# fugue-project/fugue

Measured on NVIDIA H100. Metric: transform() rows/sec, hash-partitioned (num=256) identity map, 8-col table, higher is better.
Workload: dtype int64+f64 (byte moves; u64 hash arithmetic)

## Files before the change

fugue_b200/csrc/fb_partition.cu:

```cuda
#include <stdlib.h>

#include <mutex>

#include "fb_common.cuh"

namespace {

constexpr int kBlock = 512;
constexpr int kItems = 8;
constexpr int kTile = kBlock * kItems;
constexpr int kWarps = kBlock / 32;
constexpr int kCtasPerSm = 2;

struct FbCols {
  const void* src[FB_MAX_COLS];
  void* dst[FB_MAX_COLS];
  int32_t width[FB_MAX_COLS];
  int32_t ncols;
};

struct ChunkGeom {
  int64_t nrows;
  int64_t full_rows;
  int64_t tiles_per_chunk;
  int32_t nchunks_full;
  int32_t nchunks;
};

inline ChunkGeom make_geom(int dev, int64_t nrows) {
  ChunkGeom g;
  g.nrows = nrows;
  const int64_t ntiles_full = nrows / kTile;
  g.full_rows = ntiles_full * kTile;
  const int64_t max_chunks = (int64_t)fb_sm_count(dev) * kCtasPerSm;
  g.tiles_per_chunk = ntiles_full > 0 ? (ntiles_full + max_chunks - 1) / max_chunks : 1;
  g.nchunks_full = (int32_t)((ntiles_full + g.tiles_per_chunk - 1) / g.tiles_per_chunk);
  g.nchunks = g.nchunks_full + (g.full_rows < nrows ? 1 : 0);
  return g;
}

__host__ __device__ __forceinline__ void chunk_range(const ChunkGeom& g, int c, int64_t& r0, int64_t& r1) {
  if (c < g.nchunks_full) {
    r0 = (int64_t)c * g.tiles_per_chunk * kTile;
    r1 = r0 + g.tiles_per_chunk * kTile;
    if (r1 > g.full_rows) r1 = g.full_rows;
  } else {
    r0 = g.full_rows;
    r1 = g.nrows;
  }
}
// ... 15 lines not shown
__global__ void fb_pid_kernel(FbKeys keys, FbDiv dv, int64_t nrows, uint32_t* __restrict__ out) {
  int64_t i = (int64_t)blockIdx.x * blockDim.x + threadIdx.x;
  int64_t stride = (int64_t)gridDim.x * blockDim.x;
  for (; i < nrows; i += stride) out[i] = compute_pid<kSingleU64>(keys, dv, i);
}

__global__ void fb_row_hash_kernel(FbKeys keys, int64_t nrows, uint64_t* __restrict__ out) {
  int64_t i = (int64_t)blockIdx.x * blockDim.x + threadIdx.x;
  int64_t stride = (int64_t)gridDim.x * blockDim.x;
  for (; i < nrows; i += stride) out[i] = fb_row_hash(keys, i);
}

template <int kBits>
__device__ __forceinline__ unsigned match_lanes(uint32_t v, unsigned m) {
#pragma unroll
  for (int b = 0; b < kBits; ++b) {
    const int s = (int)(v << (31 - b)) >> 31;
    const unsigned bal = __ballot_sync(0xFFFFFFFFu, s < 0);
    m &= ~(bal ^ (unsigned)s);
  }
  return m;
}

constexpr int kHistBlock = 1024;
constexpr int kHistWarps = kHistBlock / 32;
constexpr int kHistRows = kHistBlock * kItems;

template <bool kSingleU64, int kBits>
__global__ void __launch_bounds__(kHistBlock, 2)
fb_hist_kernel(FbKeys keys, FbDiv dv, uint32_t num, ChunkGeom g, int chunk0, uint32_t* __restrict__ hist) {
  extern __shared__ uint32_t s_cnt[];
  for (uint32_t i = threadIdx.x; i < (uint32_t)kHistWarps * num; i += kHistBlock) s_cnt[i] = 0;
  __syncthreads();
  int64_t row0, row1;
  chunk_range(g, chunk0 + (int)blockIdx.x, row0, row1);
  const unsigned lt = fb_lanemask_lt();
  uint32_t* my = s_cnt + (size_t)(threadIdx.x >> 5) * num;
  for (int64_t base = row0; base < row1; base += kHistRows) {
    uint32_t pid[kItems];
    const bool full = base + kHistRows <= row1;
#pragma unroll
    for (int r = 0; r < kItems; ++r) {
      int64_t row = base + (int64_t)r * kHistBlock + threadIdx.x;
      pid[r] = (full || row < row1) ? compute_pid<kSingleU64>(keys, dv, row) : 0xFFFFFFFFu;
    }
#pragma unroll
    for (int r = 0; r < kItems; ++r) {
      const bool ok = pid[r] != 0xFFFFFFFFu;
      unsigned m = match_lanes<kBits>(pid[r], __ballot_sync(0xFFFFFFFFu, ok));
      if (ok && (m & lt) == 0) my[pid[r]] += (uint32_t)__popc(m);
      __syncwarp();
    }
  }
  __syncthreads();
// ... 5 lines not shown
    out[b] = t;
  }
}

constexpr int kRankBlock = 512, kRankWarps = kRankBlock / 32;
constexpr int kRankRounds = kTile / 32;
constexpr int kRankBatch = 8;
constexpr uint32_t kMetaRank = kTile, kMetaCnt = 3 * kTile, kMetaBytes = 3 * kTile + 512;
static_assert(kRankRounds % kRankBatch == 0, "a tile is a whole number of key batches");

template <bool kSingleU64>
__device__ __forceinline__ uint32_t pid_of_key(const FbKeys& keys, const FbDiv& dv, uint64_t v) {
  if (kSingleU64) return fb_fastmod(fb_hash_single_u64(v), dv);
  return (uint32_t)(v >> keys.digit_shift) & (dv.d - 1);
}

template <bool kSingleU64, int kBits, bool kStaged>
__global__ void __launch_bounds__(kRankBlock, 2)
fb_rank_tile_kernel(FbKeys keys, FbDiv dv, uint32_t num, ChunkGeom g, uint32_t* __restrict__ hist,
                    uint8_t* __restrict__ meta) {
  __shared__ __align__(16) uint16_t s_cnt[kRankWarps * 256];
  __shared__ uint32_t s_hist[256];
  const unsigned lane = threadIdx.x & 31, warp = threadIdx.x >> 5;
  const unsigned lt = fb_lanemask_lt();
  uint16_t* __restrict__ my = s_cnt + warp * 256;
  ((uint4*)my)[lane] = make_uint4(0, 0, 0, 0);
  if (threadIdx.x < 256) s_hist[threadIdx.x] = 0;
  __syncthreads();
  int64_t row0, row1;
  chunk_range(g, (int)blockIdx.x, row0, row1);
  constexpr int64_t kStride = (int64_t)kRankWarps * kTile;
  uint32_t acc[8] = {0, 0, 0, 0, 0, 0, 0, 0};
  const unsigned long long* __restrict__ kp = (const unsigned long long*)keys.ptr[0] + lane;
  uint64_t kv[kRankBatch];
  if constexpr (kStaged) {
    if (row0 + (int64_t)warp * kTile < row1) {
#pragma unroll
      for (int b = 0; b < kRankBatch; ++b) kv[b] = __ldg(kp + row0 + (int64_t)warp * kTile + b * 32);
    }
  }
  for (int64_t t0 = row0 + (int64_t)warp * kTile; t0 < row1; t0 += kStride) {
    uint8_t* __restrict__ rec = meta + (size_t)(t0 / kTile) * kMetaBytes;
    uint8_t* __restrict__ rec_id = rec + lane;
    uint16_t* __restrict__ rec_rank = (uint16_t*)(rec + kMetaRank) + lane;
    for (int r0 = 0; r0 < kRankRounds; r0 += kRankBatch) {
      uint32_t pid[kRankBatch];
      if constexpr (kStaged) {
#pragma unroll
        for (int b = 0; b < kRankBatch; ++b) pid[b] = pid_of_key<kSingleU64>(keys, dv, kv[b]);
        const int64_t nxt = r0 + kRankBatch < kRankRounds ? t0 + (r0 + kRankBatch) * 32 : t0 + kStride;
        if (nxt < row1) {
#pragma unroll
          for (int b = 0; b < kRankBatch; ++b) kv[b] = __ldg(kp + nxt + b * 32);
// ... 5 lines not shown
      }
#pragma unroll
      for (int b = 0; b < kRankBatch; ++b) {
        const uint32_t p = pid[b];
        const unsigned m = match_lanes<kBits>(p, 0xFFFFFFFFu);
        const unsigned before = __popc(m & lt);
        const uint32_t old = my[p];
        __syncwarp();
        if (before == 0) my[p] = (uint16_t)(old + __popc(m));
        __syncwarp();
        rec_id[(r0 + b) * 32] = (uint8_t)p;
        rec_rank[(r0 + b) * 32] = (uint16_t)(old + before);
      }
    }
    const uint4 c = ((const uint4*)my)[lane];
    ((uint4*)(rec + kMetaCnt))[lane] = c;
    acc[0] += c.x & 0xFFFFu; acc[1] += c.x >> 16;
    acc[2] += c.y & 0xFFFFu; acc[3] += c.y >> 16;
    acc[4] += c.z & 0xFFFFu; acc[5] += c.z >> 16;
    acc[6] += c.w & 0xFFFFu; acc[7] += c.w >> 16;
    ((uint4*)my)[lane] = make_uint4(0, 0, 0, 0);
    __syncwarp();
  }
#pragma unroll
  for (int i = 0; i < 8; ++i)
    if (acc[i] != 0) atomicAdd(&s_hist[lane * 8 + i], acc[i]);
  __syncthreads();
  if (threadIdx.x < num) hist[(size_t)blockIdx.x * num + threadIdx.x] = s_hist[threadIdx.x];
}

__global__ void __launch_bounds__(256)
fb_scan_chunks_kernel(uint32_t* __restrict__ hist, uint32_t num, int32_t nchunks,
                      int64_t* __restrict__ totals) {
  __shared__ uint32_t s_warp[8];
  __shared__ uint32_t s_carry;
  const uint32_t b = blockIdx.x;
  const unsigned lane = threadIdx.x & 31, warp = threadIdx.x >> 5;
  if (threadIdx.x == 0) s_carry = 0;
  __syncthreads();
  for (int32_t c0 = 0; c0 < nchunks; c0 += 256) {
    int32_t c = c0 + threadIdx.x;
    uint32_t v = c < nchunks ? hist[(size_t)c * num + b] : 0;
    uint32_t x = v;
#pragma unroll
    for (int o = 1; o < 32; o <<= 1) {
      uint32_t y = __shfl_up_sync(0xFFFFFFFFu, x, o);
      if (lane >= (unsigned)o) x += y;
    }
    if (lane == 31) s_warp[warp] = x;
    __syncthreads();
    uint32_t wbase = 0;
    for (unsigned w = 0; w < warp; ++w) wbase += s_warp[w];
    uint32_t carry = s_carry;
    if (c < nchunks) hist[(size_t)c * num + b] = carry + wbase + x - v;
    __syncthreads();
    if (threadIdx.x == 255) s_carry = carry + wbase + x;
    __syncthreads();
  }
  if (threadIdx.x == 0) totals[b] = (int64_t)s_carry;
}

__global__ void __launch_bounds__(1024)
fb_scan_parts_kernel(int64_t* __restrict__ offsets, uint32_t num) {
  __shared__ int64_t s_warp[32];
  __shared__ int64_t s_carry;
  const unsigned lane = threadIdx.x & 31, warp = threadIdx.x >> 5;
  if (threadIdx.x == 0) s_carry = 0;
  __syncthreads();
  for (uint32_t b0 = 0; b0 < num; b0 += 1024) {
    uint32_t b = b0 + threadIdx.x;
    int64_t v = b < num ? offsets[b] : 0;
    int64_t x = v;
#pragma unroll
    for (int o = 1; o < 32; o <<= 1) {
      int64_t y = __shfl_up_sync(0xFFFFFFFFu, x, o);
      if (lane >= (unsigned)o) x += y;
    }
    if (lane == 31) s_warp[warp] = x;
    __syncthreads();
    int64_t wbase = 0;
    for (unsigned w = 0; w < warp; ++w) wbase += s_warp[w];
    int64_t carry = s_carry;
    if (b < num) offsets[b] = carry + wbase + x - v;
    __syncthreads();
    if (threadIdx.x == 1023) s_carry = carry + wbase + x;
    __syncthreads();
  }
  if (threadIdx.x == 0) offsets[num] = s_carry;
}

// ... 176 lines not shown
  cx.cursor = cx.delta + cx.nbp;
  cx.bin_start = cx.cursor + cx.nbp;
  cx.cnt = cx.bin_start + cx.nbp;
  cx.scanw = cx.cnt + kWarps * cx.nbp;
  cx.pid_sorted = (uint16_t*)(cx.scanw + 32);

  const int chunk = chunk0 + (int)blockIdx.x;
  int64_t chunk_row0, chunk_row1;
  chunk_range(g, chunk, chunk_row0, chunk_row1);

  for (uint32_t b = threadIdx.x; b < cx.nbp; b += kBlock)
    cx.cursor[b] = b < num ? (uint32_t)part_offsets[b] + chunk_base[(size_t)chunk * num + b] : 0u;
  for (uint32_t i = threadIdx.x; i < (uint32_t)kWarps * cx.nbp; i += kBlock) cx.cnt[i] = 0;
  __syncthreads();

  int phase = 0;
  for (int64_t tile_row0 = chunk_row0; tile_row0 < chunk_row1; tile_row0 += kTile) {
    const int64_t left = chunk_row1 - tile_row0;
    if (left >= kTile)
      scatter_tile<kSingleU64, kBits, true, kAll8>(keys, dv, num, cols, cx, tile_row0, kTile, phase);
    else
      scatter_tile<kSingleU64, kBits, false, kAll8>(keys, dv, num, cols, cx, tile_row0, (int)left, phase);
  }
}

constexpr int kSwcMaxCols = 8;
constexpr uint32_t kSwcMaxNum = 256;

__device__ __forceinline__ uint32_t smem_u32(const void* p) { return (uint32_t)__cvta_generic_to_shared(p); }

__device__ __forceinline__ void mbar_init(uint32_t bar, uint32_t count) {
  asm volatile("mbarrier.init.shared::cta.b64 [%0], %1;" ::"r"(bar), "r"(count) : "memory");
}
__device__ __forceinline__ void mbar_expect_tx(uint32_t bar, uint32_t bytes) {
  asm volatile("mbarrier.arrive.expect_tx.shared::cta.b64 _, [%0], %1;" ::"r"(bar), "r"(bytes) : "memory");
}
__device__ __forceinline__ void mbar_arrive_relaxed(uint32_t bar) {
  asm volatile("mbarrier.arrive.relaxed.cta.shared::cta.b64 _, [%0];" ::"r"(bar) : "memory");
}
__device__ __forceinline__ void mbar_wait(uint32_t bar, uint32_t parity) {
  asm volatile(
      "{\n"
      ".reg .pred p;\n"
      "FB_WAIT:\n"
      "mbarrier.try_wait.parity.shared::cta.b64 p, [%0], %1;\n"
      "@p bra FB_DONE;\n"
// ... 45 lines not shown
  uint64_t a[FB_MAX_COLS], b[FB_MAX_COLS], c[FB_MAX_COLS];
  int32_t mode[FB_MAX_COLS];
};

__device__ __forceinline__ uint64_t ws_apply_map(int mode, bool two, uint64_t x, uint64_t y, uint64_t a, uint64_t b,
                                                 uint64_t c) {
  if (mode == 1) {
    double r = __dmul_rn(__longlong_as_double((long long)a), __longlong_as_double((long long)x));
    if (two) r = __dadd_rn(r, __dmul_rn(__longlong_as_double((long long)b), __longlong_as_double((long long)y)));
    return (uint64_t)__double_as_longlong(__dadd_rn(r, __longlong_as_double((long long)c)));
  }
  if (mode == 2) return a * x + (two ? b * y : 0ULL) + c;
  return x;
}

template <int G, int RI>
__host__ __device__ inline size_t ws_book_bytes(uint32_t num, int ncols) {
  constexpr size_t kT = (size_t)kWsRankers * RI;
  const size_t nbp = nb_padded(num);
  const size_t E = (size_t)num * (G - 1);
  size_t b = 64 * 8;
  b += (size_t)ncols * E * 8;
  b += (kT + E) * 4;
  b += 5 * nbp * 4 + 64 * 4;
  b += ((E * 2 + 15) / 16) * 16;
  b += 2 * (size_t)kMetaBytes + 128;
  return b;
}

__device__ __forceinline__ void mbar_arrive(uint32_t bar) {
  asm volatile("mbarrier.arrive.shared::cta.b64 _, [%0];" ::"r"(bar) : "memory");
}
__device__ __forceinline__ void mover_sync() { asm volatile("bar.sync 1, %0;" ::"n"(kWsMovers) : "memory"); }
__device__ __forceinline__ void ranker_sync() { asm volatile("bar.sync 2, %0;" ::"n"(kWsRankers) : "memory"); }
template <uint32_t N>
__device__ __forceinline__ void setmaxnreg_dec() { asm volatile("setmaxnreg.dec.sync.aligned.u32 %0;" ::"n"(N)); }
template <uint32_t N>
__device__ __forceinline__ void setmaxnreg_inc() { asm volatile("setmaxnreg.inc.sync.aligned.u32 %0;" ::"n"(N)); }

template <int kBits, int G, int kWsRankItems, bool kMap>
__global__ void __launch_bounds__(kWsThreads, 1)
fb_scatter_ws_kernel(WsUnits units, uint32_t num, ChunkGeom g, int nstages,
                     const uint8_t* __restrict__ meta,
                     const uint32_t* __restrict__ chunk_base, const int64_t* __restrict__ part_offsets,
                     const __grid_constant__ WsMap map) {
  constexpr uint32_t T = (uint32_t)kWsRankers * kWsRankItems;
  static_assert(T == (uint32_t)kTile, "pass 1 ranks tiles of kTile rows");
  static_assert(G >= 2 && G <= 16 && (G & (G - 1)) == 0, "G must be a power of two <= 16");
  constexpr uint32_t GM = G - 1;
  constexpr uint32_t kStageBytes = T * 8;
  constexpr int kSlotRounds = ((int)T + (int)kSwcMaxNum * (G - 1) + kWsMovers - 1) / kWsMovers;
  constexpr int kEntryRoundsM = ((int)kSwcMaxNum * (G - 1) + kWsMovers - 1) / kWsMovers;
  extern __shared__ __align__(128) uint64_t smem64[];
  const uint32_t nbp = nb_padded(num);
  const uint32_t E = num * GM;
  const int grp = (int)blockIdx.x % units.ngroups;
  const int chunk_first = (int)blockIdx.x / units.ngroups, chunk_step = (int)gridDim.x / units.ngroups;
  const int u0 = grp * units.per_group;
  const int ncols = min(units.per_group, units.nunits - u0);
  uint64_t* ring = smem64;
  uint64_t* bars = ring + (size_t)nstages * T;
  uint64_t* carry = bars + 64;
  uint32_t* slotinfo = (uint32_t*)(carry + (size_t)ncols * E);
  uint32_t* wpos = slotinfo + T + E;
  uint32_t* kcnt = wpos + nbp;
  uint32_t* binfo = kcnt + nbp;
  uint32_t* wstart = binfo + nbp;
  uint32_t* wdelta = wstart + nbp;
  uint32_t* scanw = wdelta + nbp;
  uint16_t* carryinfo = (uint16_t*)(scanw + 64);
  uint8_t* metabuf = (uint8_t*)(((uintptr_t)(carryinfo + E) + 127) & ~(uintptr_t)127);

  const unsigned lane = threadIdx.x & 31, warp = threadIdx.x >> 5;
  const uint32_t bar_full = smem_u32(bars), bar_empty = smem_u32(bars + 16);
  const uint32_t bar_pid_full = smem_u32(bars + 32), bar_pid_empty = smem_u32(bars + 34);
  const uint32_t bar_slots_ready = smem_u32(bars + 36), bar_slots_free = smem_u32(bars + 37);
  const uint32_t bar_flush_done = smem_u32(bars + 38);

  if (threadIdx.x == 0) {
    for (int s = 0; s < nstages; ++s) {
      mbar_init(bar_full + 8 * s, 1);
      mbar_init(bar_empty + 8 * s, kWsMoverWarps);
    }
    for (int i = 0; i < 2; ++i) {
      mbar_init(bar_pid_full + 8 * i, 1);
      mbar_init(bar_pid_empty + 8 * i, kWsRankWarps);
    }
    mbar_init(bar_slots_ready, kWsRankWarps);
    mbar_init(bar_slots_free, kWsMoverWarps);
    mbar_init(bar_flush_done, kWsMoverWarps);
    asm volatile("fence.mbarrier_init.release.cluster;" ::: "memory");
  }
  __syncthreads();

  if (warp >= kWsMoverWarps + kWsRankWarps) {
    setmaxnreg_dec<kWsProducerRegs>();
    if (warp == kWsMoverWarps + kWsRankWarps && lane == 0) {
      const uint64_t pol = l2_policy_evict_first(), meta_pol = l2_policy_evict_last();
      const uint32_t ring_s = smem_u32(ring), meta_s = smem_u32(metabuf);
      uint32_t s = 0, ph = 0, seq = 0;
      int chunk = chunk_first;
      int64_t r0 = 0, r1 = 0, t0 = 0;
      bool have = chunk < g.nchunks_full;
      if (have) { chunk_range(g, chunk, r0, r1); t0 = r0; }
      auto load_pid = [&](int64_t row0, uint32_t q) {
        const uint32_t b = q & 1, pp = (q >> 1) & 1;
        mbar_wait(bar_pid_empty + 8 * b, pp ^ 1);
        mbar_expect_tx(bar_pid_full + 8 * b, kMetaBytes);
        tma_load_1d(meta_s + b * kMetaBytes, meta + (size_t)(row0 / T) * kMetaBytes, kMetaBytes,
                    bar_pid_full + 8 * b, meta_pol);
      };
      if (have) load_pid(t0, 0);
      while (have) {
        int nchunk = chunk;
        int64_t nr0 = r0, nr1 = r1, nt0 = t0 + T;
        bool nhave = true;
        if (nt0 >= r1) {
          nchunk = chunk + chunk_step;
          nhave = nchunk < g.nchunks_full;
          if (nhave) { chunk_range(g, nchunk, nr0, nr1); nt0 = nr0; }
        }
        if (nhave) load_pid(nt0, seq + 1);
        for (int u = u0; u < u0 + ncols; ++u) {
          mbar_wait(bar_empty + 8 * s, ph ^ 1);
          mbar_expect_tx(bar_full + 8 * s, kStageBytes);
          tma_load_1d(ring_s + s * kStageBytes, units.src[u] + t0, kStageBytes, bar_full + 8 * s, pol);
          if (++s == (uint32_t)nstages) { s = 0; ph ^= 1; }
          if constexpr (kMap) {
            if (map.src2[u] != nullptr) {
              mbar_wait(bar_empty + 8 * s, ph ^ 1);
              mbar_expect_tx(bar_full + 8 * s, kStageBytes);
              tma_load_1d(ring_s + s * kStageBytes, map.src2[u] + t0, kStageBytes, bar_full + 8 * s, pol);
              if (++s == (uint32_t)nstages) { s = 0; ph ^= 1; }
            }
          }
        }
        chunk = nchunk; r0 = nr0; r1 = nr1; t0 = nt0; have = nhave;
        ++seq;
      }
    }
    return;
  }

  if (warp >= kWsMoverWarps) {
    setmaxnreg_dec<kWsRankerRegs>();
    const unsigned rw = warp - kWsMoverWarps;
    const unsigned rtid = threadIdx.x - kWsMovers;
    uint32_t seq = 0, cseq = 0;
    for (int chunk = chunk_first; chunk < g.nchunks_full; chunk += chunk_step, ++cseq) {
      int64_t r0, r1;
      chunk_range(g, chunk, r0, r1);
      if (cseq > 0) mbar_wait(bar_flush_done, (cseq - 1) & 1);
      ranker_sync();
      for (uint32_t b = rtid; b < nbp; b += kWsRankers) {
        const uint32_t p0 = b < num ? (uint32_t)part_offsets[b] + chunk_base[(size_t)chunk * num + b] : 0u;
        wpos[b] = p0 & ~GM;
        kcnt[b] = (p0 & GM) | ((p0 & GM) << 8);
      }
      ranker_sync();
      for (int64_t t0 = r0; t0 < r1; t0 += T, ++seq) {
        const uint32_t pb = seq & 1, pph = (seq >> 1) & 1;
        mbar_wait(bar_pid_full + 8 * pb, pph);
        const uint8_t* __restrict__ rec = metabuf + pb * kMetaBytes;
        const uint32_t b = rtid;
        uint32_t n = 0, w = 0, kold = 0, phold = 0, wp_old = 0;
        if (b < num) n = ((const uint16_t*)(rec + kMetaCnt))[b];
        if (b < num) {
          const uint32_t kc = kcnt[b];
          kold = kc & 0xFFu;
          phold = kc >> 8;
          wp_old = wpos[b];
          const uint32_t end = wp_old + kold + n;
          const uint32_t aend = end & ~GM;
          if (aend > wp_old) {
            w = aend - wp_old;
            wpos[b] = aend;
            kcnt[b] = end - aend;
          } else {
            kcnt[b] = (kold + n) | (phold << 8);
          }
          binfo[b] = kold | (w << 8);
        }
        uint32_t xw = w;
#pragma unroll
        for (int o = 1; o < 32; o <<= 1) {
          const uint32_t yw = __shfl_up_sync(0xFFFFFFFFu, xw, o);
          if (lane >= (unsigned)o) xw += yw;
        }
        if (lane == 31) scanw[8 + rw] = xw;
        ranker_sync();
        uint32_t bw = xw - w;
        {
          const uint32_t tw = lane < kWsRankWarps ? scanw[8 + lane] : 0;
#pragma unroll
          for (int wi = 0; wi < kWsRankWarps; ++wi) {
            const uint32_t vw = __shfl_sync(0xFFFFFFFFu, tw, wi);
            if ((unsigned)wi < rw) bw += vw;
          }
        }
        if (seq > 0) mbar_wait(bar_slots_free, (seq - 1) & 1);
        if (b < num) {
          wstart[b] = bw;
          wdelta[b] = wp_old - bw;
        }
        if (rtid == kWsRankers - 1) scanw[40] = bw + w;
        ranker_sync();
#pragma unroll
        for (int r = 0; r < kWsRankItems; ++r) {
          const uint32_t row = r * kWsRankers + rtid;
          const uint32_t pb2 = rec[row];
          const uint32_t bi = binfo[pb2];
          const uint32_t i = (bi & 0xFFu) + ((const uint16_t*)(rec + kMetaRank))[row];
          const uint32_t ww = bi >> 8;
          if (i < ww) slotinfo[wstart[pb2] + i] = (pb2 << 16) | row;
          else carryinfo[pb2 * GM + (i - ww)] = (uint16_t)row;
        }
        __syncwarp();
        if (lane == 0) mbar_arrive_relaxed(bar_pid_empty + 8 * pb);
        if (b < num) {
#pragma unroll
          for (uint32_t i = 0; i < GM; ++i) {
            const uint32_t e = b * GM + i;
            const uint32_t desc = i < phold ? 0xFFFFu : T + e;
            if (i < kold) {
              if (i < w) slotinfo[bw + i] = (b << 16) | desc;
              else carryinfo[e] = (uint16_t)desc;
            }
            if (w + i >= kold + n) carryinfo[e] = 0xFFFFu;
          }
        }
        ranker_sync();
        if (lane == 0) mbar_arrive(bar_slots_ready);
      }
    }
    return;
  }

  setmaxnreg_inc<kWsMoverRegs>();
  uint32_t s = 0, ph = 0, seq = 0;
  for (int chunk = chunk_first; chunk < g.nchunks_full; chunk += chunk_step) {
    int64_t r0, r1;
    chunk_range(g, chunk, r0, r1);
    for (int64_t t0 = r0; t0 < r1; t0 += T, ++seq) {
      mbar_wait(bar_slots_ready, seq & 1);
      const uint32_t W = scanw[40];
      uint32_t srcd[kSlotRounds], dst[kSlotRounds];
#pragma unroll
      for (int k = 0; k < kSlotRounds; ++k) {
        const uint32_t j = k * kWsMovers + threadIdx.x;
        srcd[k] = 0xFFFFu;
        dst[k] = 0;
        if (j < W) {
          const uint32_t info = slotinfo[j];
          srcd[k] = info & 0xFFFFu;
          dst[k] = wdelta[info >> 16] + j;
        }
      }
      uint32_t csrc[kEntryRoundsM];
#pragma unroll
      for (int q = 0; q < kEntryRoundsM; ++q) {
        const uint32_t e = q * kWsMovers + threadIdx.x;
        const uint32_t d = e < E ? (uint32_t)carryinfo[e] : 0xFFFFu;
        csrc[q] = d < T ? d : 0xFFFFu;
      }
      __syncwarp();
      if (lane == 0) mbar_arrive(bar_slots_free);

      for (int u = 0; u < ncols; ++u) {
        mbar_wait(bar_full + 8 * s, ph);
        const uint64_t* __restrict__ st = ring + (size_t)s * T;
        uint64_t* __restrict__ out = units.dst[u0 + u];
        uint64_t* __restrict__ cbuf = carry + (size_t)u * E;
        uint32_t s2 = s;
        bool two = false;
        const uint64_t* __restrict__ st2 = st;
        int mode = 0;
        uint64_t ma = 0, mb = 0, mc = 0;
        if constexpr (kMap) {
          mode = map.mode[u0 + u];
          two = map.src2[u0 + u] != nullptr;
          if (two) {
            s2 = s + 1 == (uint32_t)nstages ? 0 : s + 1;
            mbar_wait(bar_full + 8 * s2, s2 == 0 ? ph ^ 1 : ph);
            st2 = ring + (size_t)s2 * T;
          }
          ma = map.a[u0 + u]; mb = map.b[u0 + u]; mc = map.c[u0 + u];
        }
        auto staged = [&](uint32_t r) -> uint64_t {
          if constexpr (kMap) return ws_apply_map(mode, two, st[r], st2[r], ma, mb, mc);
          else return st[r];
        };
#pragma unroll
// ... 3 lines not shown
          for (int k = 0; k < kMoveBatch; ++k)
            if (k0 + k < kSlotRounds && srcd[k0 + k] != 0xFFFFu)
              v[k] = srcd[k0 + k] < T ? staged(srcd[k0 + k]) : cbuf[srcd[k0 + k] - T];
#pragma unroll
          for (int k = 0; k < kMoveBatch; ++k)
            if (k0 + k < kSlotRounds && srcd[k0 + k] != 0xFFFFu) out[dst[k0 + k]] = v[k];
        }
        mover_sync();
#pragma unroll
        for (int q = 0; q < kEntryRoundsM; ++q)
          if (csrc[q] != 0xFFFFu) cbuf[q * kWsMovers + threadIdx.x] = staged(csrc[q]);
        __syncwarp();
        if (lane == 0) {
          mbar_arrive_relaxed(bar_empty + 8 * s);
          if (kMap && two) mbar_arrive_relaxed(bar_empty + 8 * s2);
        }
        if (++s == (uint32_t)nstages) { s = 0; ph ^= 1; }
        if (kMap && two) {
          if (++s == (uint32_t)nstages) { s = 0; ph ^= 1; }
        }
      }
      if (ncols == 1) mover_sync();
    }
    mover_sync();
    for (int u = 0; u < ncols; ++u) {
      uint64_t* __restrict__ out = units.dst[u0 + u];
      const uint64_t* __restrict__ cbuf = carry + (size_t)u * E;
#pragma unroll
      for (int q = 0; q < kEntryRoundsM; ++q) {
        const uint32_t e = q * kWsMovers + threadIdx.x;
        if (e < E) {
          const uint32_t b = e / GM, i = e - b * GM;
          const uint32_t kc = kcnt[b];
          if (i < (kc & 0xFFu) && i >= (kc >> 8)) out[wpos[b] + i] = cbuf[e];
        }
      }
    }
    __syncwarp();
    if (lane == 0) mbar_arrive(bar_flush_done);
  }
}

__global__ void fb_bits_to_bytes_kernel(const uint8_t* __restrict__ bits, int64_t bit_offset,
                                        int64_t nrows, uint8_t* __restrict__ out) {
  int64_t i = (int64_t)blockIdx.x * blockDim.x + threadIdx.x;
  int64_t stride = (int64_t)gridDim.x * blockDim.x;
  for (; i < nrows; i += stride) {
    int64_t j = i + bit_offset;
    out[i] = (bits[j >> 3] >> (j & 7)) & 1;
  }
}

__global__ void fb_bytes_to_bits_kernel(const uint8_t* __restrict__ bytes, int64_t nrows,
                                        uint8_t* __restrict__ out, unsigned long long* null_count) {
  int64_t nbytes = (nrows + 7) >> 3;
  int64_t i = (int64_t)blockIdx.x * blockDim.x + threadIdx.x;
  int64_t stride = (int64_t)gridDim.x * blockDim.x;
  unsigned long long nulls = 0;
  for (; i < nbytes; i += stride) {
    uint8_t v = 0;
#pragma unroll
    for (int k = 0; k < 8; ++k) {
      int64_t r = i * 8 + k;
// ... 81 lines not shown
    k.valid[i] = valid ? valid[i] : nullptr;
  }
  return 0;
}

struct PlanLayout {
  size_t hist_bytes;
  size_t pid_offset;
  size_t total_bytes;
};

PlanLayout plan_layout(const ChunkGeom& g, uint32_t num) {
  PlanLayout l;
  l.hist_bytes = (((size_t)g.nchunks * num * sizeof(uint32_t)) + 255) & ~(size_t)255;
  l.pid_offset = l.hist_bytes + 256;
  l.total_bytes = l.pid_offset + (num <= kSwcMaxNum ? (size_t)(g.full_rows / kTile) * kMetaBytes : 0) + 256;
  return l;
}

}

extern "C" {

size_t fb_partition_scratch_bytes(int dev, int64_t nrows, uint32_t num_partitions) {
  if (nrows < 0 || num_partitions == 0) return 0;
  ChunkGeom g = make_geom(dev, nrows);
  return plan_layout(g, num_partitions).total_bytes;
}

int fb_partition_ids(int dev, void* stream, int64_t nrows, int nkeys, const void* const* key_ptrs,
                     const int32_t* key_widths, const uint8_t* const* key_valid,
                     uint32_t num_partitions, uint32_t* out_pids) {
  FB_CHECK(nrows >= 0, "nrows < 0");
  FB_CHECK(num_partitions >= 1, "num_partitions must be >= 1");
  if (nrows == 0) return 0;
  FbDeviceGuard guard(dev);
  FB_CHECK(guard.ok, "cannot select device %d", dev);
  FbKeys k;
  if (int rc = fill_keys(k, nkeys, key_ptrs, key_widths, key_valid)) return rc;
  FbDiv dv = fb_make_div(num_partitions);
  int64_t blocks = (nrows + 255) / 256;
  int64_t maxb = (int64_t)fb_sm_count(dev) * 16;
  if (blocks > maxb) blocks = maxb;
  cudaStream_t st = (cudaStream_t)stream;
  if (single_u64_key(nkeys, key_widths, key_valid))
    fb_pid_kernel<true><<<(unsigned)blocks, 256, 0, st>>>(k, dv, nrows, out_pids);
// ... 28 lines not shown
  FB_CHECK(num_partitions >= 1 && num_partitions <= FB_MAX_PARTITIONS,
           "num_partitions=%u out of range [1,%d]", num_partitions, FB_MAX_PARTITIONS);
  FB_CHECK(out_part_offsets != nullptr, "out_part_offsets is NULL");
  FbDeviceGuard guard(dev);
  FB_CHECK(guard.ok, "cannot select device %d", dev);
  cudaStream_t st = (cudaStream_t)stream;
  if (nrows == 0) {
    FB_CUDA(cudaMemsetAsync(out_part_offsets, 0, sizeof(int64_t) * ((size_t)num_partitions + 1), st));
    return 0;
  }
  ChunkGeom g = make_geom(dev, nrows);
  PlanLayout l = plan_layout(g, num_partitions);
  FB_CHECK(scratch != nullptr && scratch_bytes >= l.total_bytes,
           "scratch too small: need %zu bytes, got %zu", l.total_bytes, scratch_bytes);
  FbDiv dv = fb_make_div(num_partitions);
  uint32_t* hist = (uint32_t*)scratch;
  size_t smem = (size_t)kHistWarps * num_partitions * sizeof(uint32_t);
  FB_CUDA(ensure_smem_optin(dev));
  const int bits = bits_for(num_partitions);
  int hist_chunk0 = 0;
  if (num_partitions <= kSwcMaxNum && g.nchunks_full > 0) {
    uint8_t* meta = (uint8_t*)scratch + l.pid_offset;
#define FB_LAUNCH_RANK(S, B, STAGED) \
  fb_rank_tile_kernel<S, B, STAGED><<<g.nchunks_full, kRankBlock, 0, st>>>(k, dv, num_partitions, g, hist, meta)
    if (single) {
      if (bits == 4) FB_LAUNCH_RANK(true, 4, true);
      else FB_LAUNCH_RANK(true, 8, true);
    } else if (k.digit_shift >= 0) {
      if (bits == 4) FB_LAUNCH_RANK(false, 4, true);
      else FB_LAUNCH_RANK(false, 8, true);
    } else {
      if (bits == 4) FB_LAUNCH_RANK(false, 4, false);
      else FB_LAUNCH_RANK(false, 8, false);
    }
#undef FB_LAUNCH_RANK
    FB_CUDA(cudaGetLastError());
    hist_chunk0 = g.nchunks_full;
  }
  if (hist_chunk0 < g.nchunks) {
#define FB_LAUNCH_HIST(S, B)                                                                       \
  fb_hist_kernel<S, B><<<g.nchunks - hist_chunk0, kHistBlock, smem, st>>>(k, dv, num_partitions, g, \
                                                                          hist_chunk0, hist)
    FB_DISPATCH_SB(single, bits, FB_LAUNCH_HIST);
#undef FB_LAUNCH_HIST
    FB_CUDA(cudaGetLastError());
  }
  fb_scan_chunks_kernel<<<num_partitions, 256, 0, st>>>(hist, num_partitions, g.nchunks, out_part_offsets);
  FB_CUDA(cudaGetLastError());
  fb_scan_parts_kernel<<<1, 1024, 0, st>>>(out_part_offsets, num_partitions);
  FB_CUDA(cudaGetLastError());
  return 0;
}

int fb_partition_plan(int dev, void* stream, int64_t nrows, int nkeys, const void* const* key_ptrs,
                      const int32_t* key_widths, const uint8_t* const* key_valid,
                      uint32_t num_partitions, void* scratch, size_t scratch_bytes,
                      int64_t* out_part_offsets) {
  FbKeys k;
  if (nrows == 0) {
    memset(&k, 0, sizeof(k));
    k.nkeys = 1;
    k.digit_shift = -1;
    return plan_impl(dev, stream, 0, k, false, num_partitions, scratch, scratch_bytes, out_part_offsets);
  }
  if (int rc = fill_keys(k, nkeys, key_ptrs, key_widths, key_valid)) return rc;
  return plan_impl(dev, stream, nrows, k, single_u64_key(nkeys, key_widths, key_valid), num_partitions,
                   scratch, scratch_bytes, out_part_offsets);
}

__global__ void fb_map_tail_kernel(int ncols, const void* const* __restrict__ x_ptrs, const fb_map_unit* __restrict__ maps,
                                   int64_t row0, int64_t nrows, uint64_t* __restrict__ tmp) {
  const int64_t n = nrows - row0;
  for (int64_t i = (int64_t)blockIdx.x * blockDim.x + threadIdx.x; i < n * ncols; i += (int64_t)gridDim.x * blockDim.x) {
// ... 14 lines not shown
  FB_CHECK(nrows >= 0 && nrows < ((int64_t)1 << 32), "nrows out of range");
  FB_CHECK(num_partitions >= 1 && num_partitions <= FB_MAX_PARTITIONS,
           "num_partitions=%u out of range [1,%d]", num_partitions, FB_MAX_PARTITIONS);
  FB_CHECK(ncols >= 0, "ncols < 0");
  if (nrows == 0 || ncols == 0) return 0;
  FbDeviceGuard guard(dev);
  FB_CHECK(guard.ok, "cannot select device %d", dev);
  ChunkGeom g = make_geom(dev, nrows);
  PlanLayout l = plan_layout(g, num_partitions);
  FB_CHECK(scratch != nullptr && scratch_bytes >= l.total_bytes, "scratch too small");
  FbDiv dv = fb_make_div(num_partitions);
  cudaStream_t st = (cudaStream_t)stream;
  const size_t smem = scatter_smem_bytes(num_partitions);
  FB_CUDA(ensure_smem_optin(dev));
  const int bits = bits_for(num_partitions);

  for (int c = 0; c < ncols; ++c) {
    const int w = col_widths[c];
    FB_CHECK(w == 1 || w == 2 || w == 4 || w == 8, "column %d has unsupported width %d", c, w);
    FB_CHECK(col_ptrs[c] != nullptr && out_col_ptrs[c] != nullptr, "column %d pointer is NULL", c);
  }

  const void* const* gen_src = col_ptrs;
  auto launch_generic = [&](const int* idx, int n, int chunk0, int nch) -> int {
    for (int c0 = 0; c0 < n && nch > 0; c0 += FB_MAX_COLS) {
      FbCols cols;
      memset(&cols, 0, sizeof(cols));
      cols.ncols = n - c0 < FB_MAX_COLS ? n - c0 : FB_MAX_COLS;
      bool all8 = true;
      for (int c = 0; c < cols.ncols; ++c) {
        cols.src[c] = gen_src[idx[c0 + c]];
        cols.dst[c] = out_col_ptrs[idx[c0 + c]];
        cols.width[c] = col_widths[idx[c0 + c]];
        all8 = all8 && cols.width[c] == 8;
      }
#define FB_LAUNCH_SCATTER(S, B)                                                                        \
  do {                                                                                                 \
    if (all8)                                                                                          \
      fb_scatter_kernel<S, B, true><<<nch, kBlock, smem, st>>>(k, dv, num_partitions, g, chunk0,       \
                                                               (const uint32_t*)scratch, part_offsets, cols); \
    else                                                                                               \
      fb_scatter_kernel<S, B, false><<<nch, kBlock, smem, st>>>(k, dv, num_partitions, g, chunk0,      \
                                                                (const uint32_t*)scratch, part_offsets, cols); \
  } while (0)
      FB_DISPATCH_SB(single, bits, FB_LAUNCH_SCATTER);
#undef FB_LAUNCH_SCATTER
      FB_CUDA(cudaGetLastError());
    }
    return 0;
  };

  const bool fast_ok = num_partitions <= kSwcMaxNum && g.nchunks_full > 0;
  if (maps != nullptr) {
    FB_CHECK(num_partitions <= kSwcMaxNum, "fused map needs num_partitions <= %u", kSwcMaxNum);
    FB_CHECK(tail_tmp != nullptr || g.full_rows == nrows, "fused map: tail_tmp is NULL");
    for (int c = 0; c < ncols; ++c) {
      FB_CHECK(col_widths[c] == 8 && (uintptr_t)col_ptrs[c] % 16 == 0, "fused map: column %d is not an aligned 8-byte column", c);
      FB_CHECK(maps[c].mode >= 0 && maps[c].mode <= 2, "fused map: column %d has mode %d", c, maps[c].mode);
      FB_CHECK(maps[c].src2 == nullptr || (maps[c].mode != 0 && (uintptr_t)maps[c].src2 % 16 == 0),
               "fused map: bad second operand of column %d", c);
    }
// ... 32 lines not shown
      const int lg = ngroups - g0 < groups_per_launch ? ngroups - g0 : groups_per_launch;
      const int c0 = g0 * per_group;
      const int nu = nfast - c0 < lg * per_group ? nfast - c0 : lg * per_group;
      WsUnits wu;
      WsMap wm;
      memset(&wu, 0, sizeof(wu));
      memset(&wm, 0, sizeof(wm));
      wu.nunits = nu;
      wu.per_group = per_group;
      wu.ngroups = lg;
      for (int c = 0; c < nu; ++c) {
        wu.src[c] = (const uint64_t*)col_ptrs[fast_idx[c0 + c]];
        wu.dst[c] = (uint64_t*)out_col_ptrs[fast_idx[c0 + c]];
        if (maps != nullptr) {
          const fb_map_unit& m = maps[fast_idx[c0 + c]];
          wm.src2[c] = (const uint64_t*)m.src2;
          wm.a[c] = m.a; wm.b[c] = m.b; wm.c[c] = m.c;
          wm.mode[c] = m.mode;
        }
      }
      const int64_t ctas = avail < (int64_t)lg * g.nchunks_full ? avail : (int64_t)lg * g.nchunks_full;
      const int grid = (int)(ctas / lg) * lg;
#define FB_LAUNCH_WS(B, G, M)                                                                               \
  fb_scatter_ws_kernel<B, G, kWsRankItems, M><<<grid, kWsThreads, tsmem, st>>>(                              \
      wu, num_partitions, g, nstages, pid_plane, (const uint32_t*)scratch, part_offsets, wm)
#define FB_LAUNCH_WS_G(G)                                                                                   \
  do {                                                                                                      \
    if (maps != nullptr) {                                                                                  \
      if (bits == 4) FB_LAUNCH_WS(4, G, true);                                                              \
      else FB_LAUNCH_WS(8, G, true);                                                                        \
    } else if (bits == 4) {                                                                                 \
      FB_LAUNCH_WS(4, G, false);                                                                            \
    } else {                                                                                                \
      FB_LAUNCH_WS(8, G, false);                                                                            \
    }                                                                                                       \
  } while (0)
      if (lines) FB_LAUNCH_WS_G(kWsG);
      else FB_LAUNCH_WS_G(kWsGWide);
#undef FB_LAUNCH_WS_G
#undef FB_LAUNCH_WS
      FB_CUDA(cudaGetLastError());
    }
    if (maps == nullptr)
      if (int rc = launch_generic(fast_idx, nfast, g.nchunks_full, g.nchunks - g.nchunks_full)) return rc;
  }
  if (maps != nullptr && g.full_rows < nrows) {
    FB_CHECK(ncols <= kSwcMaxCols * 8, "fused map: too many columns (%d)", ncols);
    uint8_t* base = (uint8_t*)tail_tmp;
    const size_t hdr = (((size_t)ncols * (sizeof(void*) + sizeof(fb_map_unit))) + 255) & ~(size_t)255;
    FB_CUDA(cudaMemcpyAsync(base, col_ptrs, sizeof(void*) * (size_t)ncols, cudaMemcpyHostToDevice, st));
    FB_CUDA(cudaMemcpyAsync(base + sizeof(void*) * (size_t)ncols, maps, sizeof(fb_map_unit) * (size_t)ncols,
                            cudaMemcpyHostToDevice, st));
    uint64_t* vals = (uint64_t*)(base + hdr);
    fb_map_tail_kernel<<<32, 256, 0, st>>>(ncols, (const void* const*)base,
                                           (const fb_map_unit*)(base + sizeof(void*) * (size_t)ncols), g.full_rows,
                                           nrows, vals);
    FB_CUDA(cudaGetLastError());
    const void** shifted = (const void**)alloca(sizeof(void*) * (size_t)ncols);
    int* all_idx = (int*)alloca(sizeof(int) * (size_t)ncols);
    for (int c = 0; c < ncols; ++c) {
      shifted[c] = (const uint8_t*)(vals + (size_t)c * kTile) - (size_t)g.full_rows * 8;
      all_idx[c] = c;
    }
    gen_src = shifted;
    if (int rc = launch_generic(all_idx, ncols, g.nchunks_full, g.nchunks - g.nchunks_full)) return rc;
  }
  return 0;
// ... 116 lines not shown
```

Baseline: 17.69 billion.

## Chain partition kernels with programmatic dependent launch and double-buffer ranker state

Scan, warp-specialized scatter and tail-scatter kernels are now launched with programmatic stream serialization, issuing griddepcontrol wait/launch so each kernel's prologue overlaps the previous kernel's tail. The rank kernel now also handles the partial tail chunk, which removes the separate hist kernel launch. Scatter rankers double-buffer wpos/kcnt per chunk and precompute the next chunk's start offsets, so they wait on the flush barrier later instead of stalling at each chunk boundary. Optional FB_PROBE instrumentation is added, and it is compiled out by default.

Result: no change. 17.77 billion, median of 6 (+0.5%).

```diff
diff --git a/fugue_b200/csrc/fb_partition.cu b/fugue_b200/csrc/fb_partition.cu
--- a/fugue_b200/csrc/fb_partition.cu
+++ b/fugue_b200/csrc/fb_partition.cu
@@ -1,6 +1,7 @@
 #include <stdlib.h>
 
 #include <mutex>
+#include <utility>
 
 #include "fb_common.cuh"
 
@@ -26,6 +27,26 @@
   int32_t nchunks_full;
   int32_t nchunks;
 };
+
+#ifdef FB_PROBE
+constexpr int kProbeScatter = 32, kProbeRankBase = 1024 * kProbeScatter;
+__device__ unsigned long long* fb_probe_buf;
+__device__ __forceinline__ unsigned long long probe_ns() {
+  unsigned long long t;
+  asm volatile("mov.u64 %0, %%globaltimer;" : "=l"(t));
+  return t;
+}
+#define FB_PROBE_ONLY(...) __VA_ARGS__
+#define FB_TIMED_WAIT(acc, ...)           \
+  do {                                    \
+    const long long t_ = clock64();       \
+    __VA_ARGS__;                          \
+    acc += (unsigned long long)(clock64() - t_); \
+  } while (0)
+#else
+#define FB_PROBE_ONLY(...)
+#define FB_TIMED_WAIT(acc, ...) __VA_ARGS__
+#endif
 
 inline ChunkGeom make_geom(int dev, int64_t nrows) {
   ChunkGeom g;
@@ -87,6 +108,25 @@
   return m;
 }
 
+__device__ __forceinline__ void grid_dep_wait() { asm volatile("griddepcontrol.wait;" ::: "memory"); }
+__device__ __forceinline__ void grid_dep_launch() { asm volatile("griddepcontrol.launch_dependents;" ::: "memory"); }
+
+template <typename... KArgs, typename... Args>
+cudaError_t launch_pdl(void (*kernel)(KArgs...), dim3 grid, dim3 block, size_t smem, cudaStream_t st,
+                       Args&&... args) {
+  cudaLaunchConfig_t cfg = {};
+  cfg.gridDim = grid;
+  cfg.blockDim = block;
+  cfg.dynamicSmemBytes = smem;
+  cfg.stream = st;
+  cudaLaunchAttribute attr[1];
+  attr[0].id = cudaLaunchAttributeProgrammaticStreamSerialization;
+  attr[0].val.programmaticStreamSerializationAllowed = 1;
+  cfg.attrs = attr;
+  cfg.numAttrs = 1;
+  return cudaLaunchKernelEx(&cfg, kernel, std::forward<Args>(args)...);
+}
+
 constexpr int kHistBlock = 1024;
 constexpr int kHistWarps = kHistBlock / 32;
 constexpr int kHistRows = kHistBlock * kItems;
@@ -95,6 +135,7 @@
 __global__ void __launch_bounds__(kHistBlock, 2)
 fb_hist_kernel(FbKeys keys, FbDiv dv, uint32_t num, ChunkGeom g, int chunk0, uint32_t* __restrict__ hist) {
   extern __shared__ uint32_t s_cnt[];
+  grid_dep_launch();
   for (uint32_t i = threadIdx.x; i < (uint32_t)kHistWarps * num; i += kHistBlock) s_cnt[i] = 0;
   __syncthreads();
   int64_t row0, row1;
@@ -146,13 +187,23 @@
   __shared__ __align__(16) uint16_t s_cnt[kRankWarps * 256];
   __shared__ uint32_t s_hist[256];
   const unsigned lane = threadIdx.x & 31, warp = threadIdx.x >> 5;
+  FB_PROBE_ONLY(unsigned long long* prec = fb_probe_buf + kProbeRankBase + (size_t)blockIdx.x * 32;
+                if (threadIdx.x == 0) prec[0] = probe_ns();)
   const unsigned lt = fb_lanemask_lt();
   uint16_t* __restrict__ my = s_cnt + warp * 256;
   ((uint4*)my)[lane] = make_uint4(0, 0, 0, 0);
   if (threadIdx.x < 256) s_hist[threadIdx.x] = 0;
+  grid_dep_launch();
   __syncthreads();
   int64_t row0, row1;
   chunk_range(g, (int)blockIdx.x, row0, row1);
+  if ((int)blockIdx.x == g.nchunks_full) {
+    for (int64_t row = row0 + threadIdx.x; row < row1; row += kRankBlock)
+      atomicAdd(&s_hist[compute_pid<kSingleU64>(keys, dv, row)], 1u);
+    __syncthreads();
+    if (threadIdx.x < num) hist[(size_t)blockIdx.x * num + threadIdx.x] = s_hist[threadIdx.x];
+    return;
+  }
   constexpr int64_t kStride = (int64_t)kRankWarps * kTile;
   uint32_t acc[8] = {0, 0, 0, 0, 0, 0, 0, 0};
   const unsigned long long* __restrict__ kp = (const unsigned long long*)keys.ptr[0] + lane;
@@ -204,6 +255,7 @@
     ((uint4*)my)[lane] = make_uint4(0, 0, 0, 0);
     __syncwarp();
   }
+  FB_PROBE_ONLY(if (lane == 0) prec[1 + warp] = probe_ns();)
 #pragma unroll
   for (int i = 0; i < 8; ++i)
     if (acc[i] != 0) atomicAdd(&s_hist[lane * 8 + i], acc[i]);
@@ -219,6 +271,8 @@
   const uint32_t b = blockIdx.x;
   const unsigned lane = threadIdx.x & 31, warp = threadIdx.x >> 5;
   if (threadIdx.x == 0) s_carry = 0;
+  grid_dep_wait();
+  grid_dep_launch();
   __syncthreads();
   for (int32_t c0 = 0; c0 < nchunks; c0 += 256) {
     int32_t c = c0 + threadIdx.x;
@@ -248,6 +302,8 @@
   __shared__ int64_t s_carry;
   const unsigned lane = threadIdx.x & 31, warp = threadIdx.x >> 5;
   if (threadIdx.x == 0) s_carry = 0;
+  grid_dep_wait();
+  grid_dep_launch();
   __syncthreads();
   for (uint32_t b0 = 0; b0 < num; b0 += 1024) {
     uint32_t b = b0 + threadIdx.x;
@@ -470,6 +526,7 @@
     else
       scatter_tile<kSingleU64, kBits, false, kAll8>(keys, dv, num, cols, cx, tile_row0, (int)left, phase);
   }
+  grid_dep_wait();
 }
 
 constexpr int kSwcMaxCols = 8;
@@ -561,7 +618,7 @@
   size_t b = 64 * 8;
   b += (size_t)ncols * E * 8;
   b += (kT + E) * 4;
-  b += 5 * nbp * 4 + 64 * 4;
+  b += 5 * nbp * 4 + 2 * nbp * 2 + 64 * 4;
   b += ((E * 2 + 15) / 16) * 16;
   b += 2 * (size_t)kMetaBytes + 128;
   return b;
@@ -601,13 +658,13 @@
   uint64_t* bars = ring + (size_t)nstages * T;
   uint64_t* carry = bars + 64;
   uint32_t* slotinfo = (uint32_t*)(carry + (size_t)ncols * E);
-  uint32_t* wpos = slotinfo + T + E;
-  uint32_t* kcnt = wpos + nbp;
-  uint32_t* binfo = kcnt + nbp;
+  uint32_t* wpos2 = slotinfo + T + E;
+  uint32_t* binfo = wpos2 + 2 * nbp;
   uint32_t* wstart = binfo + nbp;
   uint32_t* wdelta = wstart + nbp;
   uint32_t* scanw = wdelta + nbp;
-  uint16_t* carryinfo = (uint16_t*)(scanw + 64);
+  uint16_t* kcnt2 = (uint16_t*)(scanw + 64);
+  uint16_t* carryinfo = kcnt2 + 2 * nbp;
   uint8_t* metabuf = (uint8_t*)(((uintptr_t)(carryinfo + E) + 127) & ~(uintptr_t)127);
 
   const unsigned lane = threadIdx.x & 31, warp = threadIdx.x >> 5;
@@ -615,6 +672,8 @@
   const uint32_t bar_pid_full = smem_u32(bars + 32), bar_pid_empty = smem_u32(bars + 34);
   const uint32_t bar_slots_ready = smem_u32(bars + 36), bar_slots_free = smem_u32(bars + 37);
   const uint32_t bar_flush_done = smem_u32(bars + 38);
+  FB_PROBE_ONLY(unsigned long long* prec = fb_probe_buf + (size_t)blockIdx.x * kProbeScatter;
+                if (threadIdx.x == 0) { prec[0] = probe_ns(); prec[12] = clock64(); })
 
   if (threadIdx.x == 0) {
     for (int s = 0; s < nstages; ++s) {
@@ -635,6 +694,9 @@
   if (warp >= kWsMoverWarps + kWsRankWarps) {
     setmaxnreg_dec<kWsProducerRegs>();
     if (warp == kWsMoverWarps + kWsRankWarps && lane == 0) {
+      grid_dep_wait();
+      grid_dep_launch();
+      FB_PROBE_ONLY(unsigned long long w_empty = 0;)
       const uint64_t pol = l2_policy_evict_first(), meta_pol = l2_policy_evict_last();
       const uint32_t ring_s = smem_u32(ring), meta_s = smem_u32(metabuf);
       uint32_t s = 0, ph = 0, seq = 0;
@@ -644,7 +706,7 @@
       if (have) { chunk_range(g, chunk, r0, r1); t0 = r0; }
       auto load_pid = [&](int64_t row0, uint32_t q) {
         const uint32_t b = q & 1, pp = (q >> 1) & 1;
-        mbar_wait(bar_pid_empty + 8 * b, pp ^ 1);
+        FB_TIMED_WAIT(w_empty, mbar_wait(bar_pid_empty + 8 * b, pp ^ 1));
         mbar_expect_tx(bar_pid_full + 8 * b, kMetaBytes);
         tma_load_1d(meta_s + b * kMetaBytes, meta + (size_t)(row0 / T) * kMetaBytes, kMetaBytes,
                     bar_pid_full + 8 * b, meta_pol);
@@ -661,7 +723,7 @@
         }
         if (nhave) load_pid(nt0, seq + 1);
         for (int u = u0; u < u0 + ncols; ++u) {
-          mbar_wait(bar_empty + 8 * s, ph ^ 1);
+          FB_TIMED_WAIT(w_empty, mbar_wait(bar_empty + 8 * s, ph ^ 1));
           mbar_expect_tx(bar_full + 8 * s, kStageBytes);
           tma_load_1d(ring_s + s * kStageBytes, units.src[u] + t0, kStageBytes, bar_full + 8 * s, pol);
           if (++s == (uint32_t)nstages) { s = 0; ph ^= 1; }
@@ -677,6 +739,7 @@
         chunk = nchunk; r0 = nr0; r1 = nr1; t0 = nt0; have = nhave;
         ++seq;
       }
+      FB_PROBE_ONLY(atomicAdd(&prec[4], w_empty);)
     }
     return;
   }
@@ -686,20 +749,27 @@
     const unsigned rw = warp - kWsMoverWarps;
     const unsigned rtid = threadIdx.x - kWsMovers;
     uint32_t seq = 0, cseq = 0;
+    FB_PROBE_ONLY(unsigned long long w_pid = 0, w_free = 0, w_flush = 0;)
+    grid_dep_wait();
+    grid_dep_launch();
+    auto chunk_start = [&](int c) -> uint32_t {
+      return c < g.nchunks_full && rtid < num ? (uint32_t)part_offsets[rtid] + chunk_base[(size_t)c * num + rtid] : 0u;
+    };
+    uint32_t p_next = chunk_start(chunk_first);
     for (int chunk = chunk_first; chunk < g.nchunks_full; chunk += chunk_step, ++cseq) {
       int64_t r0, r1;
       chunk_range(g, chunk, r0, r1);
-      if (cseq > 0) mbar_wait(bar_flush_done, (cseq - 1) & 1);
-      ranker_sync();
-      for (uint32_t b = rtid; b < nbp; b += kWsRankers) {
-        const uint32_t p0 = b < num ? (uint32_t)part_offsets[b] + chunk_base[(size_t)chunk * num + b] : 0u;
-        wpos[b] = p0 & ~GM;
-        kcnt[b] = (p0 & GM) | ((p0 & GM) << 8);
+      FB_PROBE_ONLY(if (rtid == 0 && cseq < 16) prec[16 + cseq] = probe_ns();)
+      uint32_t* __restrict__ wpos = wpos2 + (cseq & 1) * nbp;
+      uint16_t* __restrict__ kcnt = kcnt2 + (cseq & 1) * nbp;
+      if (rtid < num) {
+        wpos[rtid] = p_next & ~GM;
+        kcnt[rtid] = (uint16_t)((p_next & GM) | ((p_next & GM) << 8));
       }
-      ranker_sync();
+      p_next = chunk_start(chunk + chunk_step);
       for (int64_t t0 = r0; t0 < r1; t0 += T, ++seq) {
         const uint32_t pb = seq & 1, pph = (seq >> 1) & 1;
-        mbar_wait(bar_pid_full + 8 * pb, pph);
+        FB_TIMED_WAIT(w_pid, mbar_wait(bar_pid_full + 8 * pb, pph));
         const uint8_t* __restrict__ rec = metabuf + pb * kMetaBytes;
         const uint32_t b = rtid;
         uint32_t n = 0, w = 0, kold = 0, phold = 0, wp_old = 0;
@@ -714,9 +784,9 @@
           if (aend > wp_old) {
             w = aend - wp_old;
             wpos[b] = aend;
-            kcnt[b] = end - aend;
+            kcnt[b] = (uint16_t)(end - aend);
           } else {
-            kcnt[b] = (kold + n) | (phold << 8);
+            kcnt[b] = (uint16_t)((kold + n) | (phold << 8));
           }
           binfo[b] = kold | (w << 8);
         }
@@ -737,7 +807,7 @@
             if ((unsigned)wi < rw) bw += vw;
           }
         }
-        if (seq > 0) mbar_wait(bar_slots_free, (seq - 1) & 1);
+        if (seq > 0) FB_TIMED_WAIT(w_free, mbar_wait(bar_slots_free, (seq - 1) & 1));
         if (b < num) {
           wstart[b] = bw;
           wdelta[b] = wp_old - bw;
@@ -770,18 +840,31 @@
         }
         ranker_sync();
         if (lane == 0) mbar_arrive(bar_slots_ready);
+        if (t0 == r0 && cseq > 0) FB_TIMED_WAIT(w_flush, mbar_wait(bar_flush_done, (cseq - 1) & 1));
       }
     }
+    FB_PROBE_ONLY(if (lane == 0) { atomicAdd(&prec[5], w_pid); atomicAdd(&prec[6], w_free); atomicAdd(&prec[7], w_flush); })
     return;
   }
 
   setmaxnreg_inc<kWsMoverRegs>();
-  uint32_t s = 0, ph = 0, seq = 0;
-  for (int chunk = chunk_first; chunk < g.nchunks_full; chunk += chunk_step) {
+  grid_dep_wait();
+  grid_dep_launch();
+  FB_PROBE_ONLY(if (threadIdx.x == 0) prec[1] = probe_ns();)
+  uint32_t s = 0, ph = 0, seq = 0, cseq = 0;
+  FB_PROBE_ONLY(unsigned long long w_full = 0, w_ready = 0, t_flush = 0;)
+  for (int chunk = chunk_first; chunk < g.nchunks_full; chunk += chunk_step, ++cseq) {
     int64_t r0, r1;
     chunk_range(g, chunk, r0, r1);
+    const uint32_t* __restrict__ wpos = wpos2 + (cseq & 1) * nbp;
+    const uint16_t* __restrict__ kcnt = kcnt2 + (cseq & 1) * nbp;
     for (int64_t t0 = r0; t0 < r1; t0 += T, ++seq) {
-      mbar_wait(bar_slots_ready, seq & 1);
+      FB_TIMED_WAIT(w_ready, mbar_wait(bar_slots_ready, seq & 1));
+      FB_PROBE_ONLY(if (threadIdx.x == 0 && t_flush != 0) {
+        prec[10] += probe_ns() - t_flush;
+        prec[11] += 1;
+        t_flush = 0;
+      })
       const uint32_t W = scanw[40];
       uint32_t srcd[kSlotRounds], dst[kSlotRounds];
 #pragma unroll
@@ -806,7 +889,8 @@
       if (lane == 0) mbar_arrive(bar_slots_free);
 
       for (int u = 0; u < ncols; ++u) {
-        mbar_wait(bar_full + 8 * s, ph);
+        FB_TIMED_WAIT(w_full, mbar_wait(bar_full + 8 * s, ph));
+        FB_PROBE_ONLY(if (threadIdx.x == 0 && seq == 0 && u == 0) prec[2] = probe_ns();)
         const uint64_t* __restrict__ st = ring + (size_t)s * T;
         uint64_t* __restrict__ out = units.dst[u0 + u];
         uint64_t* __restrict__ cbuf = carry + (size_t)u * E;
@@ -856,6 +940,7 @@
       }
       if (ncols == 1) mover_sync();
     }
+    FB_PROBE_ONLY(if (threadIdx.x == 0) t_flush = probe_ns();)
     mover_sync();
     for (int u = 0; u < ncols; ++u) {
       uint64_t* __restrict__ out = units.dst[u0 + u];
@@ -873,6 +958,8 @@
     __syncwarp();
     if (lane == 0) mbar_arrive(bar_flush_done);
   }
+  FB_PROBE_ONLY(if (lane == 0) { atomicAdd(&prec[8], w_full); atomicAdd(&prec[9], w_ready); }
+                if (threadIdx.x == 0) { prec[3] = probe_ns(); prec[13] = clock64(); })
 }
 
 __global__ void fb_bits_to_bytes_kernel(const uint8_t* __restrict__ bits, int64_t bit_offset,
@@ -1000,6 +1087,13 @@
 
 extern "C" {
 
+#ifdef FB_PROBE
+int fb_probe_set(void* buf) {
+  FB_CUDA(cudaMemcpyToSymbol(fb_probe_buf, &buf, sizeof(buf)));
+  return 0;
+}
+#endif
+
 size_t fb_partition_scratch_bytes(int dev, int64_t nrows, uint32_t num_partitions) {
   if (nrows < 0 || num_partitions == 0) return 0;
   ChunkGeom g = make_geom(dev, nrows);
@@ -1074,7 +1168,7 @@
   if (num_partitions <= kSwcMaxNum && g.nchunks_full > 0) {
     uint8_t* meta = (uint8_t*)scratch + l.pid_offset;
 #define FB_LAUNCH_RANK(S, B, STAGED) \
-  fb_rank_tile_kernel<S, B, STAGED><<<g.nchunks_full, kRankBlock, 0, st>>>(k, dv, num_partitions, g, hist, meta)
+  fb_rank_tile_kernel<S, B, STAGED><<<g.nchunks, kRankBlock, 0, st>>>(k, dv, num_partitions, g, hist, meta)
     if (single) {
       if (bits == 4) FB_LAUNCH_RANK(true, 4, true);
       else FB_LAUNCH_RANK(true, 8, true);
@@ -1087,7 +1181,7 @@
     }
 #undef FB_LAUNCH_RANK
     FB_CUDA(cudaGetLastError());
-    hist_chunk0 = g.nchunks_full;
+    hist_chunk0 = g.nchunks;
   }
   if (hist_chunk0 < g.nchunks) {
 #define FB_LAUNCH_HIST(S, B)                                                                       \
@@ -1097,10 +1191,9 @@
 #undef FB_LAUNCH_HIST
     FB_CUDA(cudaGetLastError());
   }
-  fb_scan_chunks_kernel<<<num_partitions, 256, 0, st>>>(hist, num_partitions, g.nchunks, out_part_offsets);
-  FB_CUDA(cudaGetLastError());
-  fb_scan_parts_kernel<<<1, 1024, 0, st>>>(out_part_offsets, num_partitions);
-  FB_CUDA(cudaGetLastError());
+  FB_CUDA(launch_pdl(fb_scan_chunks_kernel, dim3(num_partitions), dim3(256), 0, st, hist, num_partitions, g.nchunks,
+                     out_part_offsets));
+  FB_CUDA(launch_pdl(fb_scan_parts_kernel, dim3(1), dim3(1024), 0, st, out_part_offsets, num_partitions));
   return 0;
 }
 
@@ -1161,7 +1254,7 @@
   }
 
   const void* const* gen_src = col_ptrs;
-  auto launch_generic = [&](const int* idx, int n, int chunk0, int nch) -> int {
+  auto launch_generic = [&](const int* idx, int n, int chunk0, int nch, bool pdl = false) -> int {
     for (int c0 = 0; c0 < n && nch > 0; c0 += FB_MAX_COLS) {
       FbCols cols;
       memset(&cols, 0, sizeof(cols));
@@ -1175,7 +1268,13 @@
       }
 #define FB_LAUNCH_SCATTER(S, B)                                                                        \
   do {                                                                                                 \
-    if (all8)                                                                                          \
+    if (pdl && all8)                                                                                   \
+      FB_CUDA(launch_pdl(fb_scatter_kernel<S, B, true>, dim3(nch), dim3(kBlock), smem, st, k, dv,      \
+                         num_partitions, g, chunk0, (const uint32_t*)scratch, part_offsets, cols));    \
+    else if (pdl)                                                                                      \
+      FB_CUDA(launch_pdl(fb_scatter_kernel<S, B, false>, dim3(nch), dim3(kBlock), smem, st, k, dv,     \
+                         num_partitions, g, chunk0, (const uint32_t*)scratch, part_offsets, cols));    \
+    else if (all8)                                                                                     \
       fb_scatter_kernel<S, B, true><<<nch, kBlock, smem, st>>>(k, dv, num_partitions, g, chunk0,       \
                                                                (const uint32_t*)scratch, part_offsets, cols); \
     else                                                                                               \
@@ -1254,8 +1353,8 @@
       const int64_t ctas = avail < (int64_t)lg * g.nchunks_full ? avail : (int64_t)lg * g.nchunks_full;
       const int grid = (int)(ctas / lg) * lg;
 #define FB_LAUNCH_WS(B, G, M)                                                                               \
-  fb_scatter_ws_kernel<B, G, kWsRankItems, M><<<grid, kWsThreads, tsmem, st>>>(                              \
-      wu, num_partitions, g, nstages, pid_plane, (const uint32_t*)scratch, part_offsets, wm)
+  FB_CUDA(launch_pdl(fb_scatter_ws_kernel<B, G, kWsRankItems, M>, dim3(grid), dim3(kWsThreads), tsmem, st,    \
+                     wu, num_partitions, g, nstages, pid_plane, (const uint32_t*)scratch, part_offsets, wm))
 #define FB_LAUNCH_WS_G(G)                                                                                   \
   do {                                                                                                      \
     if (maps != nullptr) {                                                                                  \
@@ -1271,10 +1370,9 @@
       else FB_LAUNCH_WS_G(kWsGWide);
 #undef FB_LAUNCH_WS_G
 #undef FB_LAUNCH_WS
-      FB_CUDA(cudaGetLastError());
     }
     if (maps == nullptr)
-      if (int rc = launch_generic(fast_idx, nfast, g.nchunks_full, g.nchunks - g.nchunks_full)) return rc;
+      if (int rc = launch_generic(fast_idx, nfast, g.nchunks_full, g.nchunks - g.nchunks_full, true)) return rc;
   }
   if (maps != nullptr && g.full_rows < nrows) {
     FB_CHECK(ncols <= kSwcMaxCols * 8, "fused map: too many columns (%d)", ncols);
```
